# DrQuestion/monica

Hardware: AMD Instinct MI355X
Metric: reads/sec classified (higher is better)
Workload: dtype u32/u64 integer; int16 pairs in the alignment kernels (int32 / int8 in the long-call and literal ones); float32 islands: overlap ratio, MAPQ

## Files before the change

### include/monica_amd.h

```cpp
#ifndef MONICA_AMD_H
#define MONICA_AMD_H

#include <stdint.h>
#include <stddef.h>

#ifdef __cplusplus
extern "C" {
#endif

#define MNC_OK               0
#define MNC_ERR_ARG         (-1)
#define MNC_ERR_IO          (-2)
#define MNC_ERR_FORMAT      (-3)
#define MNC_ERR_NOMEM       (-4)
#define MNC_ERR_HIP         (-5)
#define MNC_ERR_NODEVICE    (-6)
#define MNC_ERR_UNSUPPORTED (-7)
#define MNC_ERR_RANGE       (-8)

#define MNC_UNMAPPED   (-1)
#define MNC_AMBIGUOUS  (-2)
#define MNC_SKIPPED    (-3)

typedef struct mnc_index  mnc_index;
// ... 96 lines not shown
#define MNC_STAGE_DP_POST     14
#define MNC_STAGE_DP_FILL     15
#define MNC_STAGE_DP_FILL_T1  16
#define MNC_STAGE_DP_FILL_T2  17
#define MNC_STAGE_DP_FILL_T3  18
#define MNC_STAGE_DP_EXT      19
#define MNC_STAGE_DP_FILL_TM  20
#define MNC_STAGE_DP_LFILL    21
#define MNC_N_STAGES          22
int mnc_engine_set_profiling(mnc_engine *eng, int on);
int mnc_engine_set_debug(mnc_engine *eng, int mode);
int mnc_engine_get_timings(mnc_engine *eng, double *ms, int64_t *launches, int reset);
const char *mnc_stage_name(int stage);
const char *mnc_stage_kernel(int stage);
int mnc_engine_get_counters(mnc_engine *eng, int64_t *c, int n);

int mnc_index_set_host_tables(mnc_index *idx, int on);
int mnc_index_set_region_bits(mnc_index *idx, int bits);
int mnc_engine_dump_tables(mnc_engine *eng, void *dst, int64_t cap_bytes, int64_t *n_bytes);

#define MNC_DUMP_MINIMIZERS 1
#define MNC_DUMP_MZ_OFFSETS 2
#define MNC_DUMP_ANCHORS    3
#define MNC_DUMP_AN_OFFSETS 4
#define MNC_DUMP_CHAIN_F    5
#define MNC_DUMP_CHAIN_P    6
#define MNC_DUMP_CHAIN_V    7
#define MNC_DUMP_REGS       8
#define MNC_DUMP_REG_OFFSETS 9
#define MNC_DUMP_REP_LEN    10
// ... 74 lines not shown
```

### monica_amd/_capi.py

```python
import ctypes as C
import os

import numpy as np

_HERE = os.path.dirname(os.path.abspath(__file__))
os.environ.setdefault("OMP_WAIT_POLICY", "passive")
LIB_PATH = os.environ.get("MONICA_AMD_LIB") or os.path.join(_HERE, "libmonica_amd.so")

OK = 0
ERR_ARG, ERR_IO, ERR_FORMAT, ERR_NOMEM, ERR_HIP, ERR_NODEVICE, ERR_UNSUPPORTED, ERR_RANGE = range(-1, -9, -1)
UNMAPPED = -1
AMBIGUOUS = -2
SKIPPED = -3

HIT_DTYPE = np.dtype([("rid", "<i4"), ("mapq", "<i4"), ("nm", "<i4"), ("mlen", "<i4")])
REG_DTYPE = np.dtype([("id", "<i4"), ("parent", "<i4"), ("rid", "<i4"), ("rev", "<i4"),
                      ("rs", "<i4"), ("re", "<i4"), ("qs", "<i4"), ("qe", "<i4"),
                      ("score", "<i4"), ("score0", "<i4"), ("cnt", "<i4"), ("as", "<i4"),
                      ("mlen", "<i4"), ("blen", "<i4"), ("subsc", "<i4"), ("n_sub", "<i4"),
                      ("mapq", "<i4"), ("hash", "<u4"),
                      ("dp_score", "<i4"), ("dp_max", "<i4"), ("dp_max2", "<i4"), ("n_ambi", "<i4"),
                      ("n_cigar", "<i4"), ("flags", "<i4")])
MZ_DTYPE = np.dtype([("hash", "<u4"), ("pos_strand", "<u4")])
ANCHOR_DTYPE = np.dtype([("x", "<u8"), ("y", "<u8")])
# ... 10 lines not shown
CONTRACT_DP, CONTRACT_CHAIN = 0, 1
MAX_READ_LEN = (1 << 20) - 1
MAX_READ_LEN_WIDE = (1 << 24) - 1
MAX_READS_WIDE = 1 << 16

EXPORTS = [
    "mnc_strerror", "mnc_last_error", "mnc_device_count", "mnc_device_name", "mnc_device_mem_info",
    "mnc_index_build", "mnc_index_build_mem", "mnc_index_build_device", "mnc_index_build_mem_device", "mnc_index_save", "mnc_index_save_mmi", "mnc_index_load", "mnc_index_free",
    "mnc_index_info", "mnc_index_contig_name", "mnc_index_contig_len", "mnc_index_contig_genome",
    "mnc_index_genome_name", "mnc_index_genome_len", "mnc_index_dump", "mnc_index_set_mid_occ",
    "mnc_engine_create", "mnc_engine_destroy", "mnc_engine_stream", "mnc_engine_device_bytes", "mnc_index_device_bytes", "mnc_engine_set_index",
    "mnc_classify_batch", "mnc_engine_prefetch", "mnc_engine_prefetch_cancel", "mnc_classify_device", "mnc_engine_sync", "mnc_engine_fetch_hits",
    "mnc_counts", "mnc_best_hit",
    "mnc_engine_set_profiling", "mnc_engine_set_debug", "mnc_engine_set_contract", "mnc_engine_set_long_reads", "mnc_index_set_host_tables", "mnc_index_set_region_bits", "mnc_engine_dump_tables",
    "mnc_comm_unique_id", "mnc_comm_init_rank", "mnc_comm_destroy", "mnc_comm_count", "mnc_allreduce_counts", "mnc_allgather_summaries", "mnc_shard_summary", "mnc_merge_summaries", "mnc_engine_get_timings", "mnc_stage_name", "mnc_stage_kernel",
    "mnc_engine_get_counters", "mnc_engine_dump",
    "mnc_fastq_open", "mnc_fastq_close", "mnc_fastq_next", "mnc_fastq_detach_batch", "mnc_fastq_remaining", "mnc_fastq_bases", "mnc_fastq_offsets",
    "mnc_fastq_quals", "mnc_fastq_title", "mnc_fastq_route",
    "mnc_hitmap_create", "mnc_hitmap_load", "mnc_hitmap_save", "mnc_hitmap_free", "mnc_hitmap_size",
    "mnc_hitmap_update", "mnc_hitmap_n_names", "mnc_hitmap_name", "mnc_host_alloc", "mnc_host_free", "mnc_host_set_io_workers",
    "mnc_synth_genome", "mnc_synth_diverge", "mnc_synth_reads", "mnc_synth_reads_device", "mnc_version",
]


class IndexInfo(C.Structure):
    _fields_ = [("k", C.c_int32), ("w", C.c_int32), ("n_contigs", C.c_int32), ("n_genomes", C.c_int32),
                ("mid_occ", C.c_int32), ("reserved", C.c_int32), ("n_keys", C.c_int64),
                ("n_occ", C.c_int64), ("total_len", C.c_int64), ("table_slots", C.c_int64),
                ("device_bytes", C.c_int64)]


# ... 52 lines not shown
    sig("mnc_engine_destroy", None, [vp])
    sig("mnc_engine_stream", vp, [vp])
    sig("mnc_engine_prefetch", i32, [vp, vp, vp, u32, C.POINTER(C.c_int)])
    sig("mnc_engine_prefetch_cancel", i32, [vp])
    sig("mnc_engine_set_index", i32, [vp, vp])
    sig("mnc_engine_device_bytes", i32, [vp, C.POINTER(C.c_int64)])
    sig("mnc_index_device_bytes", i32, [vp, i32, C.POINTER(C.c_int64)])
    sig("mnc_classify_batch", i32, [vp, vp, vp, u32, i32, vp, vp, vp])
    sig("mnc_classify_device", i32, [vp, vp, vp, u32, i64, i32, i32, vp, vp, vp, vp])
    sig("mnc_engine_sync", i32, [vp])
    sig("mnc_engine_fetch_hits", i32, [vp, vp, vp, i64, C.POINTER(i64)])
    sig("mnc_counts", i32, [vp, vp, vp, vp, u32, i32, vp])
    sig("mnc_best_hit", i32, [vp, i32, C.POINTER(i32)])
    sig("mnc_engine_set_profiling", i32, [vp, i32])
    sig("mnc_engine_set_debug", i32, [vp, i32])
    sig("mnc_index_set_host_tables", i32, [vp, i32])
    sig("mnc_index_set_region_bits", i32, [vp, i32])
    sig("mnc_engine_dump_tables", i32, [vp, vp, C.c_int64, vp])
    sig("mnc_engine_set_contract", i32, [vp, i32])
    sig("mnc_engine_set_long_reads", i32, [vp, i32])
    sig("mnc_comm_unique_id", i32, [vp])
    sig("mnc_comm_init_rank", i32, [vp, i32, i32, C.POINTER(vp)])
    sig("mnc_comm_destroy", i32, [vp])
    sig("mnc_comm_count", i32, [vp, C.POINTER(i32)])
    sig("mnc_allreduce_counts", i32, [vp, i32, vp, vp])
    sig("mnc_allgather_summaries", i32, [vp, vp, C.c_size_t, vp, vp])
    sig("mnc_shard_summary", i32, [vp, vp, vp, i64, i32, vp, vp])
    sig("mnc_merge_summaries", i32, [vp, i32, i64, vp, vp, vp, vp, vp])
    sig("mnc_engine_get_timings", i32, [vp, vp, vp, i32])
    sig("mnc_stage_name", cp, [i32])
# ... 318 lines not shown
        ln = np.zeros(N_STAGES, dtype=np.int64)
        check(lib().mnc_engine_get_timings(self._h, ms.ctypes.data, ln.ctypes.data, 1 if reset else 0))
        names = [lib().mnc_stage_name(s).decode() for s in range(N_STAGES)]
        return {names[s]: (float(ms[s]), int(ln[s])) for s in range(N_STAGES)}

    def counters(self):
        c = np.zeros(24, dtype=np.int64)
        check(lib().mnc_engine_get_counters(self._h, c.ctypes.data, 24))
        keys = ["minimizers", "probe_hits", "anchors", "chains", "regions", "gated_hits", "ambiguous_reads", "batch_redone",
                "dp_segments", "dp_fill_tier1", "dp_fill_tier2", "dp_fill_handed_back",
                "dp_fill_steps_t1", "dp_fill_steps_t2", "dp_fill_steps_t3", "dp_ext_cell_steps",
                "dp_literal_big", "dp_literal_mid", "dp_long_gaps", "dp_literal_big_handed_back", "dp_long_extensions", "dp_fill_tier3",
                "dp_fill_tier_mid", "dp_fill_steps_tm"]
        return dict(zip(keys, (int(x) for x in c)))

    def dump(self, what, dtype):
        n = C.c_int64(0)
        rc = lib().mnc_engine_dump(self._h, what, None, 0, C.byref(n))
        if rc not in (OK, ERR_RANGE):
            check(rc)
        buf = np.zeros(max(n.value, 1), dtype=np.uint8)
        check(lib().mnc_engine_dump(self._h, what, buf.ctypes.data, len(buf), C.byref(n)))
        return buf[:n.value].view(dtype).copy()


def best_hit(hits):
    arr = np.zeros(len(hits), dtype=HIT_DTYPE)
    for i, (nm, mlen) in enumerate(hits):
        arr[i]["nm"], arr[i]["mlen"] = nm, mlen
    out = C.c_int(0)
# ... 139 lines not shown
```

### monica_amd/csrc/engine.hip

```cpp
#include <hip/hip_runtime.h>
#include <algorithm>
#include <cmath>
#include <cstdio>
#include <cstring>
#include <cstdlib>
#include <new>
#include <vector>

#include "device.h"
#include <atomic>
#include <thread>

#include "scan.h"

namespace mnc {

void launch_pack(const Batch &B, hipStream_t st);
void launch_sketch(const Batch &B, hipStream_t st);
void launch_partition(const Batch &B, hipStream_t st);
int partition_prepare();
void launch_probe(const Batch &B, hipStream_t st);
void launch_collect(const Batch &B, hipStream_t st);
void launch_expand_sort(const Batch &B, const uint32_t *lists, const ClassSpans &spans, int NM, hipStream_t st);
int expand_sort_prepare(int max_nm);
void launch_backtrack(const Batch &B, const uint32_t *read_list, uint32_t n_list, hipStream_t st);
void launch_bin_reads(const Batch &B, const ChainClasses &C, uint32_t *cls_count, uint32_t *cls_list, hipStream_t st);
void launch_chain_dp_ring(const Batch &B, const uint32_t *lists, const ClassSpans &spans, int stress, hipStream_t st);
void launch_chain_tail(const Batch &B, const uint32_t *lists, const ClassSpans &spans, int NM, hipStream_t st);
size_t chain_tail_lds_bytes(int NM);
int chain_tail_prepare(size_t max_lds);

static const ChainClasses CHAIN_CLASSES = { 22, { 64, 128, 192, 256, 320, 384, 448, 512, 576, 640, 768, 896, 1024, 1280, 1536, 1792, 2048, 2560,
                                                  3072, 4096, 6144, 8192 } };
void launch_regions(const Batch &B, void *regx, uint64_t *k64a, uint64_t *k64b, mnc_hit_t *gated, hipStream_t st);
void launch_regions_post(const Batch &B, mnc_reg_t *work, void *regx, uint64_t *k64a, int32_t *tmp, mnc_hit_t *gated, hipStream_t st);
void launch_dp_gather(const Batch &B, hipStream_t st);
int dp_gather_long_prepare(int lds_anchors);
void launch_dp_gather_long(const Batch &B, const uint32_t *lists, const ClassSpans &spans, int lds_anchors, hipStream_t st);
void launch_dp_round(const Batch &B, int first, hipStream_t st);
void launch_dp_round_end(const Batch &B, hipStream_t st);
int dp_plan_prepare();
void launch_dp_plan(const Batch &B, const int32_t *work_list, unsigned max_work, int wave_form, int state_max, long long p_max, int cig_max,
                    long long big_state, long long big_p, long long big_cig, long long huge_state, long long huge_p, long long huge_cig, hipStream_t st);
size_t dp_align_ws_bytes(long long state_max, long long p_max, long long cig_max);
int dp_align_prepare(int lds_bytes);
int dp_stitch_prepare();
size_t dp_inv_ws_words(int max_gap);
void launch_dp_inv(const Batch &B, const int32_t *work_list, int32_t *next_list, int32_t *ws, int n_wg, hipStream_t st);
size_t dp_stitch_pool_slack(int n_wg);
void launch_dp_align(const Batch &B, uint8_t *ws, int n_wg, long long state_max, long long p_max, long long cig_max,
// ... 50 lines not shown
                                                             const int64_t *chunk_off_bm, int64_t *q_off)
{
	const uint32_t c = blockIdx.x, b = threadIdx.x, PB_N = blockDim.x;
	const uint32_t t0 = c * HC_TILES, t1 = min(n_tiles, t0 + HC_TILES);
	int64_t run = chunk_off_bm[(size_t)b * n_chunks + c];
	for (uint32_t t = t0; t < t1; ++t) {
		q_off[(size_t)t * PB_N + b] = run;
		run += hist_tm[(size_t)t * PB_N + b];
	}
	if (c == 0 && b == 0) q_off[(size_t)n_tiles * PB_N] = chunk_off_bm[(size_t)PB_N * n_chunks];
}

struct MailItem { const void *src; uint32_t dst_word, n_words; };
constexpr int MAIL_MAX = 8;
struct MailList { MailItem it[MAIL_MAX]; int n; };
__global__ __launch_bounds__(64) void mnc_mail(MailList L, uint32_t *host_box)
{
	for (int k = 0; k < L.n; ++k) {
		const uint32_t *s = static_cast<const uint32_t*>(L.it[k].src);
		for (uint32_t i = threadIdx.x; i < L.it[k].n_words; i += 64) host_box[L.it[k].dst_word + i] = s[i];
	}
	__threadfence_system();
}

struct Buf {
	void *p = nullptr;
	size_t cap = 0;
	int ensure(size_t bytes)
	{
		if (bytes <= cap) return MNC_OK;
		if (p) { (void)hipFree(p); p = nullptr; cap = 0; }
		size_t want = bytes + bytes / 8 + 256;
		hipError_t e = hipMalloc(&p, want);
		if (e != hipSuccess) { p = nullptr; set_error("hipMalloc(%zu) failed: %s", want, hipGetErrorString(e)); return MNC_ERR_NOMEM; }
		cap = want;
		return MNC_OK;
	}
// ... 244 lines not shown
	const int64_t *pf_offsets = nullptr;
	uint32_t pf_n = 0;
	int64_t pf_total = 0;
	Buf packed, mz, hits, hist_tm, q_off, qrec, bhits, bhit_cnt;
	size_t q_cap_override = 0;
	Buf ambig, skip, mz_cnt, hit_cnt, rep_len, an_cnt, an_off, n_chain, n_reg, scan_sums, hit_off, best_mlen, hist_sums, hist_offs;
	Buf a, f, p, v, t, u;
	Buf chains_tmp, regs, regx, k64a, k64b, tmp_i32, gated, hits_csr;
	Buf stats, cls_count, cls_list;
	int contract = MNC_CONTRACT_DP;
	Buf ca, ca_cnt, chain_dst, regdp, segs, cig_seg, cig_reg, dp_ctr, work_a, work_b, big_list, huge_list, reg_cnt, regs2;
	SharedWs *ws = nullptr;
	Buf fill1, fill2, fill3, fill_mid, fill_fb, plan_long, extp, mid_list, lfill, lext, bigfb, ext1, ext2, ext3, ext4, gen_list;
	size_t seg_cap_override = 0, cig_cap_override = 0;
	uint32_t *mailbox = nullptr;
	int last_redos = 0;
	long long prev_wide_calls = 0;
	int slot_pad = 2;
	Buf inv_ws;
	int cur_max_read_len = 0;
	int long_reads = 0;
	bool cur_wide = false;
	bool have_merged = false;
	std::vector<int64_t> merged_off;
	std::vector<mnc_hit_t> merged_hits;
	int64_t merged_ctr[24]{};
	int debug = 0;
	Batch B{};
	bool have_batch = false;
	int64_t last_total_anchors = 0, last_total_hits = -1;
// ... 156 lines not shown
	if (rc) { mnc_engine_destroy(e); return rc; }
	hipError_t he = hipSetDevice(device);
	int least = 0, greatest = 0;
	if (he == hipSuccess) {
		if (hipDeviceGetStreamPriorityRange(&least, &greatest) != hipSuccess) least = greatest = 0;
		he = hipStreamCreateWithPriority(&e->stream, hipStreamNonBlocking, greatest);
	}
	for (int k = 0; k < mnc_engine::N_SIDE && he == hipSuccess; ++k) {
		he = k < 3 ? hipStreamCreateWithFlags(&e->side[k], hipStreamNonBlocking) : hipStreamCreateWithPriority(&e->side[k], hipStreamNonBlocking, greatest);
		if (he == hipSuccess) he = hipEventCreateWithFlags(&e->ev_join[k], hipEventDisableTiming);
	}
	if (he == hipSuccess) he = hipEventCreateWithFlags(&e->ev_fork, hipEventDisableTiming);
	if (he == hipSuccess) he = hipEventCreateWithFlags(&e->ev_lfill, hipEventDisableTiming);
	if (he == hipSuccess) he = hipStreamCreateWithPriority(&e->copy_stream, hipStreamNonBlocking, least);
	if (he == hipSuccess) he = hipEventCreateWithFlags(&e->ev_prefetch, hipEventDisableTiming);
	if (he == hipSuccess) he = hipHostMalloc((void**)&e->mailbox, 1024, hipHostMallocDefault);
	if (he != hipSuccess) { set_error("stream creation failed: %s", hipGetErrorString(he)); mnc_engine_destroy(e); return MNC_ERR_HIP; }
	for (int s = 0; s < MNC_N_STAGES; ++s) for (int k = 0; k < 2; ++k) (void)hipEventCreate(&e->ev[s][k]);
	std::vector<int32_t> gap(GAP_LUT);
	const float avg_span = (float)idx->k;
	for (int dd = 0; dd < GAP_LUT; ++dd) {
		int lg = 0;
		for (uint32_t v = (uint32_t)dd; v >>= 1;) ++lg;
		gap[dd] = (int)(dd * .01 * avg_span) + (dd ? lg >> 1 : 0);
	}
	rc = e->gap_lut.ensure(GAP_LUT * 4);
	if (!rc) rc = logf_tables(e, 1 << 21);
	if (!rc) rc = e->dp_ctr.ensure(64 * 8);
	if (!rc) rc = dp_align_prepare(DP_LDS_BYTES);
	if (!rc) rc = e->stats.ensure(16 * 8);
	if (!rc) rc = e->cls_count.ensure((MAX_CHAIN_CLASSES + 1) * 4 + 64);
// ... 110 lines not shown
	e->contract = contract;
	return MNC_OK;
}

extern "C" int mnc_engine_set_long_reads(mnc_engine *e, int on)
{
	if (!e) return MNC_ERR_ARG;
	e->long_reads = on != 0;
	return MNC_OK;
}

extern "C" int mnc_engine_set_debug(mnc_engine *e, int on)
{
	if (!e) return MNC_ERR_ARG;
	e->debug = on;
	return MNC_OK;
}

extern "C" int mnc_engine_get_timings(mnc_engine *e, double *ms, int64_t *launches, int reset)
{
	if (!e) return MNC_ERR_ARG;
	for (int s = 0; s < MNC_N_STAGES; ++s) {
		if (ms) ms[s] = e->ms[s];
		if (launches) launches[s] = e->launches[s];
		if (reset) e->ms[s] = 0, e->launches[s] = 0;
	}
	return MNC_OK;
}

namespace {
// ... 55 lines not shown
	launch_dp_ext(B, 32, B.ext_list1, 16, 18, B.fill_fb, 12, e->ws->ext_p.as<uint8_t>(), DP_WG_EXT, s1);
	launch_dp_ext(B, 64, B.ext_list2, 17, 19, B.fill_fb, 12, e->ws->ext_p.as<uint8_t>(), DP_WG_EXT, s1);
	launch_dp_ext(B, 128, B.ext_list3, 24, 26, B.fill_fb, 12, e->ws->ext_p.as<uint8_t>(), DP_WG_EXT / 2, s1);
	launch_dp_ext(B, 256, B.ext_list4, 25, 27, B.fill_fb, 12, e->ws->ext_p.as<uint8_t>(), DP_WG_EXT / 4, s1);
	mark(MNC_STAGE_DP_EXT, 1);
	if (serial) {
		launch_dp_lext(B, B.lext_list, 62, 63, B.fill_fb, 12, e->ws->lext_p.as<uint8_t>(), DP_WG_LEXT, s0);
		long_passes(s0);
	}
	launch_dp_align(B, e->ws->dp_ws.as<uint8_t>(), 2 * DP_WG_SMALL, DP_STATE_SMALL, DP_P_SMALL, DP_CIG_SMALL, DP_LDS0_STATE, DP_LDS0_P, DP_LDS0_CIG, 0, s2);
}
static void align_rest(const Batch &B, mnc_engine *e, hipStream_t st)
{
	launch_dp_align(B, e->ws->dp_ws.as<uint8_t>(), DP_WG_SMALL, DP_STATE_SMALL, DP_P_SMALL, DP_CIG_SMALL, DP_LDS_BYTES, 0, 0, 2, st);
	launch_dp_align(B, e->ws->dp_ws_big.as<uint8_t>(), (dp_align_long_packed(B) && !(e->debug & 0x10000)) ? 64 : DP_WG_BIG, DP_STATE_BIG, DP_P_BIG, DP_CIG_BIG, DP_LDS_BYTES, 0, 0, 4, st);
}

static int classify_once(mnc_engine *e, const uint8_t *d_bases, const int64_t *d_offsets,
                         uint32_t n_reads, int64_t total_bases, int min_mapq,
                         int32_t *d_assign, mnc_hit_t *d_best, int32_t *d_nhits, int64_t *d_counts, int *overflowed)
{
	hipStream_t st = e->stream;
	const mnc_index *idx = e->idx;
	*overflowed = 0;
	const size_t nr = (size_t)n_reads, nb = (size_t)total_bases;
	const int pb_bits = e->didx->pb_bits;
	const size_t PB_N = (size_t)1 << pb_bits, PS_TILES = (size_t)(e->cur_wide ? PS_TILES_MIN / 2 : PS_TILES_MIN);
	const size_t n_tiles = (nr + PT_READS - 1) / PT_READS, n_super = (n_tiles + PS_TILES - 1) / PS_TILES;
	size_t q_cap = nb / 3 + 4096;
	if (e->q_cap_override > q_cap) q_cap = e->q_cap_override < nb + 4096 ? e->q_cap_override : nb + 4096;
// ... 41 lines not shown
		while ((1LL << rb) < (int64_t)idx->contig_name.size()) ++rb;
		while ((1LL << pb) < longest) ++pb;
		const bool fits = 1 + rb + pb + 21 <= 64;
		B.rid_bits = fits ? rb : 0, B.rpos_bits = fits ? pb : 0;
	}
	const MapParams &P = idx->par;
	B.min_cnt = P.min_cnt, B.min_sc = P.min_chain_score, B.bw = P.bw, B.max_gap = P.max_gap, B.max_skip = P.max_chain_skip;
	B.max_iter = P.max_chain_iter, B.best_n = P.best_n, B.seed = P.seed, B.max_join_long = P.max_join_long;
	B.max_join_short = P.max_join_short, B.min_join_flank_sc = P.min_join_flank_sc, B.mask_level = P.mask_level;
	B.pri_ratio = P.pri_ratio, B.min_join_flank_ratio = P.min_join_flank_ratio;
	B.gap_lut = e->gap_lut.as<int32_t>(), B.logf_lut = e->logf_lut.as<float>(), B.logf_a_lut = e->logf_a_lut.as<float>(), B.logf_n = e->logf_n;
	B.debug_route = (e->debug >> 17 & 15) | ((e->debug >> 22 & 1) << 4) | ((e->debug >> 5 & 1) << 5)
	              | ((e->debug >> 6 & 1) << 6) | ((e->debug >> 7 & 1) << 7)
	              | ((e->debug >> 3 & 1) << 8) | ((e->debug & 1) << 9)
	              | (((unsigned)e->debug >> 31 & 1) << 10);
	B.fill_pred = (e->debug >> 8 & 0xff) ? (e->debug >> 8 & 0xff) : 32;
	B.fill_pred_mid = (e->debug >> 24 & 0x7f) ? (e->debug >> 24 & 0x7f) : 34;
	B.fill_pred_auto = !(e->debug >> 8 & 0xff) && !(e->debug >> 24 & 0x7f) && P.a == 2 && P.b == 4 && P.q == 4 && P.e == 2 &&
	                   P.q2 == 24 && P.e2 == 1 && !getenv("MNC_FILL_PRED_FIXED");
	B.contract = e->contract, B.seq4 = e->didx->seq4, B.seq_off = e->didx->seq_off;
	B.sc_a = P.a, B.sc_b = P.b, B.gap_q = P.q, B.gap_e = P.e, B.gap_q2 = P.q2, B.gap_e2 = P.e2, B.sc_ambi = P.sc_ambi;
	B.zdrop = P.zdrop, B.zdrop_inv = P.zdrop_inv, B.end_bonus = P.end_bonus, B.min_dp_max = P.min_dp_max, B.min_ksw_len = P.min_ksw_len;
	B.max_sw_mat = P.max_sw_mat;
	B.packed = e->packed.as<uint32_t>(), B.ambig = e->ambig.as<uint32_t>(), B.skip = e->skip.as<uint32_t>(), B.mz = e->mz.as<uint2>(), B.hits = e->hits.as<HitRec>();
	B.mz_cnt = e->mz_cnt.as<int32_t>(), B.hit_cnt = e->hit_cnt.as<int32_t>(), B.rep_len = e->rep_len.as<int32_t>();
	B.an_cnt = e->an_cnt.as<int64_t>(), B.an_off = e->an_off.as<int64_t>(), B.n_chain = e->n_chain.as<int32_t>(), B.n_reg = e->n_reg.as<int32_t>(), B.best_mlen = e->best_mlen.as<int32_t>();
	B.n_tiles = (uint32_t)n_tiles, B.n_super = (uint32_t)n_super;
	B.hist_tm = e->hist_tm.as<uint32_t>(), B.q_off = e->q_off.as<int64_t>(), B.qrec = e->qrec.as<uint64_t>();
	B.q_cap = (int64_t)q_cap, B.bhits = e->bhits.as<HitRec>(), B.bhit_cnt = e->bhit_cnt.as<uint32_t>();
	B.overflow = reinterpret_cast<uint32_t*>(e->stats.as<int64_t>() + 8);
	B.assign = d_assign, B.best = d_best, B.nhits = d_nhits ? d_nhits : e->out_nhits.as<int32_t>(), B.counts = d_counts;
	B.stats = e->stats.as<int64_t>();

	HIP_TRY(hipMemsetAsync(B.ambig, 0, (nr + 1) * 4, st));
	HIP_TRY(hipMemsetAsync(B.skip, 0, (nr + 1) * 4, st));
	HIP_TRY(hipMemsetAsync(B.packed + nb / 16, 0, 16, st));
	HIP_TRY(hipMemsetAsync(B.overflow, 0, 8, st));

	{ StageTimer t(e, MNC_STAGE_PACK);   launch_pack(B, st); }
	{ StageTimer t(e, MNC_STAGE_SKETCH); launch_sketch(B, st); }
	{
		StageTimer t(e, MNC_STAGE_PARTITION);
		{
			const uint32_t n_chunks = (uint32_t)((n_tiles + HC_TILES - 1) / HC_TILES);
			uint32_t *sums_bm = e->hist_sums.as<uint32_t>();
			int64_t *off_bm = e->hist_offs.as<int64_t>();
			hipLaunchKernelGGL(mnc_hist_chunk_sums, dim3(n_chunks), dim3((unsigned)PB_N), 0, st, B.hist_tm, (uint32_t)n_tiles, n_chunks, sums_bm);
			exclusive_scan(ScanInPlain<uint32_t>{sums_bm}, (int64_t)n_chunks * PB_N, off_bm, e->scan_sums.as<int64_t>(), st);
			hipLaunchKernelGGL(mnc_hist_offsets, dim3(n_chunks), dim3((unsigned)PB_N), 0, st, B.hist_tm, (uint32_t)n_tiles, n_chunks, off_bm, B.q_off);
		}
		launch_partition(B, st);
	}
	{ StageTimer t(e, MNC_STAGE_PROBE);   launch_probe(B, st); }
	{ StageTimer t(e, MNC_STAGE_COLLECT); launch_collect(B, st); }
	HIP_TRY(hipGetLastError());
	int64_t total_anchors = 0, total_q = 0;
	uint32_t cls_count[MAX_CHAIN_CLASSES + 1] = {0}, overflow = 0;
	{
		StageTimer t(e, MNC_STAGE_SORT);
		exclusive_scan(ScanInPlain<int64_t>{B.an_cnt}, (int64_t)n_reads, B.an_off, e->scan_sums.as<int64_t>(), st);
		HIP_TRY(hipMemsetAsync(e->cls_count.p, 0, (MAX_CHAIN_CLASSES + 1) * 4, st));
		launch_bin_reads(B, CHAIN_CLASSES, e->cls_count.as<uint32_t>(), e->cls_list.as<uint32_t>(), st);
		MailList ml;
		ml.n = 4;
		ml.it[0] = { B.an_off + n_reads, 0, 2 }, ml.it[1] = { B.q_off + n_tiles * PB_N, 2, 2 };
		ml.it[2] = { e->cls_count.p, 4, (uint32_t)(MAX_CHAIN_CLASSES + 1) }, ml.it[3] = { B.overflow, 4 + MAX_CHAIN_CLASSES + 1, 1 };
		hipLaunchKernelGGL(mnc_mail, dim3(1), dim3(64), 0, st, ml, e->mailbox);
		HIP_TRY(hipStreamSynchronize(st));
		memcpy(&total_anchors, e->mailbox, 8), memcpy(&total_q, e->mailbox + 2, 8);
		memcpy(cls_count, e->mailbox + 4, (MAX_CHAIN_CLASSES + 1) * 4);
		overflow = e->mailbox[4 + MAX_CHAIN_CLASSES + 1];
	}
	if (overflow || total_q > (int64_t)q_cap) {
		e->q_cap_override = (size_t)total_q + (size_t)total_q / 8 + 4096;
		*overflowed = 1;
		return MNC_OK;
	}
	if (total_anchors < 0 || total_anchors >= (1LL << 31) * 16) { set_error("anchor count %lld out of range", (long long)total_anchors); return MNC_ERR_UNSUPPORTED; }
	e->last_total_anchors = total_anchors;
	const size_t na = (size_t)total_anchors + 4, ns = (size_t)total_anchors / 3 + 4, nsr = ns + nr * (size_t)e->slot_pad;
	ENS(a, na * sizeof(Anchor));
	ENS(f, na * 4); ENS(p, na * 4); ENS(v, na * 4); ENS(t, na * 4);
	ENS(u, na * 8);
// ... 91 lines not shown
		ENSW(dp_ws, ws_small * DP_WG_SMALL * 2); ENSW(dp_ws_big, ws_big * DP_WG_BIG); ENSW(dp_ws_bigfb, ws_big * DP_WG_BIGFB); ENSW(dp_ws_huge, ws_huge * DP_WG_HUGE); ENS2(huge_list, seg_cap * 4); ENSW(dp_ws_mid, ws_small * DP_WG_MID); ENS2(mid_list, seg_cap * 4); ENS2(lfill, seg_cap * 4); ENSW(lfill_p, dp_lfill_p_slot() * DP_WG_LFILL); ENS2(lext, seg_cap * 4); ENS2(bigfb, seg_cap * 4); ENSW(lext_p, dp_lext_p_slot() * DP_WG_LEXT);
		ENS2(plan_long, (nr * 4 + 1024) * 4);
		ENS2(fill1, seg_cap * 4); ENS2(fill2, seg_cap * 4); ENS2(fill3, seg_cap * 4); ENS2(fill_mid, seg_cap * 4); ENS2(fill_fb, seg_cap * 4); ENSW(fill_p, dp_fillp_slot() * DP_WG_FILL); ENSW(fill_cig, dp_fillp_cig_slot() * DP_WG_FILL); ENS2(extp, seg_cap * 4 * 8); ENSW(extp_p, dp_extp_slot() * DP_WG_EXT); ENSW(extp_cig, dp_extp_cig_slot() * DP_WG_EXT); ENS2(ext1, seg_cap * 4); ENS2(ext2, seg_cap * 4); ENS2(ext3, seg_cap * 4); ENS2(ext4, seg_cap * 4); ENS2(gen_list, seg_cap * 4); ENSW(ext_p, dp_fill_p_slot() * DP_WG_EXT);
#undef ENS2
		if (rc2) return rc2;
		B.ca = e->ca.as<Anchor>(), B.ca_cnt = e->ca_cnt.as<int32_t>(), B.chain_dst = e->chain_dst.as<int32_t>(), B.regdp = e->regdp.as<RegDP>();
		B.segs = e->segs.as<Seg>(), B.seg_cap = (int64_t)seg_cap, B.cig_seg = e->cig_seg.as<uint32_t>(), B.cig_reg = e->cig_reg.as<uint32_t>();
		B.cig_seg_cap = (int64_t)cig_cap, B.cig_reg_cap = (int64_t)cig_reg_cap, B.dp_ctr = e->dp_ctr.as<unsigned long long>();
		B.big_list = e->big_list.as<int32_t>(), B.huge_list = e->huge_list.as<int32_t>(), B.reg_cnt = e->reg_cnt.as<int32_t>();
		B.plan_long_list = e->plan_long.as<int32_t>(), B.plan_long_cap = (long long)(nr * 4 + 1024);
		B.fill_list1 = e->fill1.as<int32_t>(), B.fill_list2 = e->fill2.as<int32_t>(), B.fill_list3 = e->fill3.as<int32_t>(), B.fill_list_mid = e->fill_mid.as<int32_t>(), B.fill_fb = e->fill_fb.as<int32_t>();
		B.ext_list1 = e->ext1.as<int32_t>(), B.ext_list2 = e->ext2.as<int32_t>(), B.ext_list3 = e->ext3.as<int32_t>(), B.ext_list4 = e->ext4.as<int32_t>(), B.gen_list = e->gen_list.as<int32_t>(), B.extp_list = e->extp.as<int32_t>(), B.mid_list = e->mid_list.as<int32_t>(), B.lfill_list = e->lfill.as<int32_t>(), B.lext_list = e->lext.as<int32_t>(), B.bigfb_list = e->bigfb.as<int32_t>();
		B.lds0_state = DP_LDS0_STATE, B.lds0_p = DP_LDS0_P, B.lds0_cig = DP_LDS0_CIG;
		int32_t *lists[2] = { e->work_a.as<int32_t>(), e->work_b.as<int32_t>() };
		B.next_list = lists[0];
		HIP_TRY(hipMemsetAsync(e->dp_ctr.p, 0, 64 * 8, st));
		{ StageTimer t(e, MNC_STAGE_REGIONS);   launch_regions(B, e->regx.p, e->k64a.as<uint64_t>(), e->k64b.as<uint64_t>(), e->gated.as<mnc_hit_t>(), st); }
		{
			StageTimer t(e, MNC_STAGE_DP_PLAN);
			launch_dp_gather(B, st);
			int c0 = 0;
			while (c0 < CHAIN_CLASSES.n && CHAIN_CLASSES.nm[c0] <= 1024) ++c0;
			ClassSpans sp;
			sp.n = CHAIN_CLASSES.n + 1 - c0, sp.stride = (uint32_t)n_reads, sp.start[0] = 0;
			for (int c = c0; c <= CHAIN_CLASSES.n; ++c) sp.start[c - c0 + 1] = sp.start[c - c0] + cls_count[c];
			launch_dp_gather_long(B, e->cls_list.as<uint32_t>() + (size_t)c0 * n_reads, sp, CHAIN_CLASSES.nm[CHAIN_CLASSES.n - 1], st);
		}
		unsigned max_work = (unsigned)nsr;
		const int long_reads = (e->debug & 0x10) ? 2 : (e->debug & 0x800000) ? 0 : n_reads <= 4096 ? 2
		                     : (e->cur_max_read_len <= 0 || e->cur_max_read_len > 6144) ? 1 : 0;
		for (int round = 0;; ++round) {
			const int32_t *work = lists[round & 1];
			int32_t *next = lists[(round + 1) & 1];
			B.next_list = next;
			launch_dp_round(B, round == 0, st);
			if (round == 0) {
				{ StageTimer t(e, MNC_STAGE_DP_PLAN);   launch_dp_plan(B, work, max_work, long_reads, (int)DP_STATE_SMALL, DP_P_SMALL, (int)DP_CIG_SMALL, DP_STATE_BIG, DP_P_BIG, DP_CIG_BIG, DP_STATE_HUGE, DP_P_HUGE, DP_CIG_HUGE, st); }
				{
					StageTimer t(e, MNC_STAGE_DP_FILL);
					if (int rcf = fork()) return rcf;
					if (e->debug & 0x10000) align_round(B, e, e->side[0], e->side[0], e->side[0], e->side[0], e->side[0]);
					else align_round(B, e, e->side[0], e->side[1], st, e->side[2], e->side[3]);
					if (int rcj = join()) return rcj;
				}
				{
					StageTimer t(e, MNC_STAGE_DP_ALIGN);
					align_rest(B, e, st);
				}
				{ StageTimer t(e, MNC_STAGE_DP_STITCH); launch_dp_stitch(B, work, next, (e->debug & 0x200000) ? 0 : e->cur_max_read_len > 0 ? e->cur_max_read_len : 8192, DP_WG_STITCH, st); }
			} else {
// ... 1 lines not shown
				if (int rcf = fork()) return rcf;
				if (e->debug & 0x10000) align_round(B, e, e->side[0], e->side[0], e->side[0], e->side[0], e->side[0]);
				else align_round(B, e, e->side[0], e->side[1], st, e->side[2], e->side[3]);
				if (int rcj = join()) return rcj;
				align_rest(B, e, st);
				launch_dp_stitch(B, work, next, (e->debug & 0x200000) ? 0 : e->cur_max_read_len > 0 ? e->cur_max_read_len : 8192, DP_WG_STITCH, st);
				launch_dp_inv(B, work, next, e->inv_ws.as<int32_t>(), (int)std::min<unsigned>(DP_WG_INV, max_work), st);
			}
			launch_dp_round_end(B, st);
			unsigned long long ctr[6] = {0};
			{
				MailList ml;
				ml.n = 3;
				ml.it[0] = { e->dp_ctr.p, 0, 12 };
				ml.it[1] = { e->dp_ctr.as<unsigned long long>() + 6, 12, 2 }, ml.it[2] = { e->dp_ctr.as<unsigned long long>() + 58, 14, 2 };
				hipLaunchKernelGGL(mnc_mail, dim3(1), dim3(64), 0, st, ml, e->mailbox);
				HIP_TRY(hipStreamSynchronize(st));
				memcpy(ctr, e->mailbox, sizeof(ctr));
				if (round == 0 && n_reads >= 4096) {
					unsigned long long big = 0, huge = 0;
					memcpy(&big, e->mailbox + 12, 8), memcpy(&huge, e->mailbox + 14, 8);
					e->prev_wide_calls = (long long)(big + huge);
				}
			}
			if (ctr[4] != 0) {
				if (ctr[4] >= 9) { set_error("a gap between two seeds is too large for the alignment workspace"); return MNC_ERR_UNSUPPORTED; }
				if (ctr[4] == 5) {
					e->slot_pad = e->slot_pad * 4;
					*overflowed = 2;
					return MNC_OK;
				}
				e->seg_cap_override = na + 2 * ns + 1024;
				e->cig_cap_override = cig_cap * 4;
				*overflowed = 2;
				return MNC_OK;
			}
			if (ctr[5] == 0) break;
			if (round > 256) { set_error("base-level alignment does not settle"); return MNC_ERR_HIP; }
			max_work = (unsigned)ctr[5];
		}
		{ StageTimer t(e, MNC_STAGE_DP_POST); launch_regions_post(B, e->regs2.as<mnc_reg_t>(), e->regx.p, e->k64a.as<uint64_t>(), e->tmp_i32.as<int32_t>(), e->gated.as<mnc_hit_t>(), st); }
	} else {
		StageTimer t(e, MNC_STAGE_REGIONS);
		launch_regions(B, e->regx.p, e->k64a.as<uint64_t>(), e->k64b.as<uint64_t>(), e->gated.as<mnc_hit_t>(), st);
	}
	HIP_TRY(hipGetLastError());
	e->have_batch = true;
	return MNC_OK;
}

extern "C" int mnc_classify_device(mnc_engine *e, const uint8_t *d_bases, const int64_t *d_offsets,
                                   uint32_t n_reads, int64_t total_bases, int max_read_len, int min_mapq,
                                   int32_t *d_assign, mnc_hit_t *d_best, int32_t *d_nhits, int64_t *d_counts)
{
	if (!e || !d_offsets || !d_assign || (total_bases > 0 && !d_bases) || total_bases < 0) return MNC_ERR_ARG;
	if (((uintptr_t)d_bases & 15u) != 0) { set_error("d_bases must be 16-byte aligned"); return MNC_ERR_ARG; }
// ... 6 lines not shown
	if (wide && n_reads > (uint32_t)WIDE_MAX_READS) { set_error("at most 2^16 reads in a call with reads of 2^20 bases or more (wide query records hold a 16-bit read ordinal)"); return MNC_ERR_UNSUPPORTED; }
	if (total_bases >= (1LL << 40)) return MNC_ERR_UNSUPPORTED;
	HIP_TRY(hipSetDevice(e->device));
	e->have_batch = false, e->last_total_hits = -1, e->have_merged = false, e->cur_wide = wide;
	const int64_t logf_want = wide ? std::min<int64_t>((int64_t)e->idx->par.a * max_read_len + 1024, INT32_MAX / 8) : 1 << 21;
	if (logf_want > e->logf_n) {
		HIP_TRY(hipStreamSynchronize(e->stream));
		if (int lrc = logf_tables(e, (int)logf_want)) return lrc;
	}
	if (n_reads == 0) {
		memset(&e->B, 0, sizeof(e->B));
		e->have_batch = true, e->last_total_anchors = 0;
		return MNC_OK;
	}
	int overflowed = 0, q_redone = 0, dp_redone = 0;
	e->cur_max_read_len = max_read_len, e->last_redos = 0;
	int rc = MNC_OK;
	for (;;) {
		rc = classify_once(e, d_bases, d_offsets, n_reads, total_bases, min_mapq, d_assign, d_best, d_nhits, d_counts, &overflowed);
		if (rc || !overflowed) break;
		++e->last_redos;
		if (overflowed == 1 && ++q_redone > 1) { set_error("query record budget exceeded twice"); rc = MNC_ERR_NOMEM; break; }
		if (overflowed == 2 && ++dp_redone > 6) { set_error("segment / CIGAR pools of the alignment stage exceeded after %d enlargements", dp_redone - 1); rc = MNC_ERR_NOMEM; break; }
	}
	return rc;
}

extern "C" int mnc_engine_prefetch(mnc_engine *e, const uint8_t *bases, const int64_t *offsets, uint32_t n_reads, int *started)
{
	if (!e || !offsets || !started) return MNC_ERR_ARG;
	*started = 0;
// ... 363 lines not shown
```

### monica_amd/csrc/k_post.hip

```cpp
#include "device.h"

namespace mnc {

__device__ __forceinline__ uint64_t mix64(uint64_t key)
{
	key = ~key + (key << 21);
	key = key ^ key >> 24;
	key = (key + (key << 3)) + (key << 8);
	key = key ^ key >> 14;
	key = (key + (key << 2)) + (key << 4);
	key = key ^ key >> 28;
	key = key + (key << 31);
	return key;
}

__device__ __forceinline__ uint32_t wang32(uint32_t key)
{
	key += ~(key << 15);
	key ^=  (key >> 10);
	key +=  (key << 3);
	key ^=  (key >> 6);
	key += ~(key << 11);
	key ^=  (key >> 16);
	return key;
// ... 400 lines not shown
					d.read = (int32_t)rd, d.order = i << 8, d.state = 1;
					B.regdp[slot + i] = d;
					B.next_list[w0 + i] = (int32_t)(slot + i);
				}
			}
		}
	} else if (dp) B.ca_cnt[rd] = 0;
	if (dp) { B.reg_cnt[rd] = n_regs; return; }
	B.n_reg[rd] = n_regs;
	B.assign[rd] = assign;
	if (B.best) B.best[rd] = best;
	B.nhits[rd] = nhits;
	B.best_mlen[rd] = best.mlen;
}

__global__ __launch_bounds__(64) void mnc_regions_post(Batch B, mnc_reg_t *work_all, RegX *regx_all, uint64_t *k64a_all,
                                                       int32_t *tmp_all, mnc_hit_t *gated_all)
{
	const uint32_t rd = blockIdx.x * blockDim.x + threadIdx.x;
	if (rd >= B.n_reads) return;
	int32_t assign = MNC_UNMAPPED, nhits = 0;
	mnc_hit_t best;
	best.rid = best.mapq = best.nm = best.mlen = 0;
	const int n0 = B.reg_cnt[rd];
	int n_regs = 0;
	if (n0 > 0) {
		const int64_t slot = reg_slot(B, rd);
		mnc_reg_t *src = B.regs + slot, *r = work_all + slot;
		RegX *ex = regx_all + slot;
		uint64_t *ka = k64a_all + slot;
		int32_t *w = tmp_all + slot * 4, *tmp = w + n0;
		mnc_hit_t *gated = gated_all + slot;
		for (int i = 0; i < n0; ++i) w[i] = i;
// ... 41 lines not shown
		for (int i = 0; i < n_regs; ++i) src[i] = r[i], B.regdp[slot + i].cig_off = (int64_t)ex[i].x0, B.regdp[slot + i].n_cigar = r[i].n_cigar;
	}
	if (B.skip[rd]) {
		assign = MNC_SKIPPED, nhits = 0;
		memset(&best, 0, sizeof(best));
	}
	B.n_reg[rd] = n_regs;
	B.assign[rd] = assign;
	if (B.best) B.best[rd] = best;
	B.nhits[rd] = nhits;
	B.best_mlen[rd] = best.mlen;
}

constexpr int CT_THREADS = 256, CT_READS = 4096, CT_LDS_BINS = 3 * 1024;

__global__ __launch_bounds__(CT_THREADS) void mnc_count_taxa(Batch B)
{
	__shared__ unsigned long long s_bins[CT_LDS_BINS];
	const int n_bins = B.n_genomes * 3;
	const bool in_lds = n_bins <= CT_LDS_BINS;
	if (in_lds) {
		for (int k = threadIdx.x; k < n_bins; k += CT_THREADS) s_bins[k] = 0;
		__syncthreads();
	}
	unsigned long long *bins = in_lds ? s_bins : (unsigned long long*)B.counts;
	const uint32_t lo = blockIdx.x * CT_READS;
	const uint32_t hi = min(B.n_reads, lo + CT_READS);
	for (uint32_t rd = lo + threadIdx.x; rd < hi; rd += CT_THREADS) {
		const int a = B.assign[rd];
		if (a < 0) continue;
		const int g = B.contig_genome[a];
		atomicAdd(&bins[g * 3 + 0], 1ULL);
// ... 13 lines not shown
	const uint32_t rd = blockIdx.x * blockDim.x + threadIdx.x;
	if (rd >= B.n_reads) return;
	const int n = B.nhits[rd];
	if (n == 0) return;
	const mnc_hit_t *src = gated_all + reg_slot(B, rd);
	mnc_hit_t *dst = out + hit_off[rd];
	for (int i = 0; i < n; ++i) dst[i] = src[i];
}

void launch_regions(const Batch &B, void *regx, uint64_t *k64a, uint64_t *k64b, mnc_hit_t *gated, hipStream_t st)
{
	if (B.n_reads == 0) return;
	hipLaunchKernelGGL(mnc_regions_decide, dim3((B.n_reads + 63) / 64), dim3(64), 0, st, B,
	                   reinterpret_cast<RegX*>(regx), k64a, k64b, gated);
	if (B.counts && B.contract != MNC_CONTRACT_DP)
		hipLaunchKernelGGL(mnc_count_taxa, dim3((B.n_reads + CT_READS - 1) / CT_READS), dim3(CT_THREADS), 0, st, B);
}

void launch_regions_post(const Batch &B, mnc_reg_t *work, void *regx, uint64_t *k64a, int32_t *tmp, mnc_hit_t *gated, hipStream_t st)
{
	if (B.n_reads == 0) return;
	hipLaunchKernelGGL(mnc_regions_post, dim3((B.n_reads + 63) / 64), dim3(64), 0, st, B, work,
	                   reinterpret_cast<RegX*>(regx), k64a, tmp, gated);
	if (B.counts) hipLaunchKernelGGL(mnc_count_taxa, dim3((B.n_reads + CT_READS - 1) / CT_READS), dim3(CT_THREADS), 0, st, B);
}

void launch_gather_hits(const Batch &B, const mnc_hit_t *gated, const int64_t *hit_off, mnc_hit_t *out, hipStream_t st)
{
	if (B.n_reads == 0) return;
	hipLaunchKernelGGL(mnc_gather_hits, dim3((B.n_reads + 255) / 256), dim3(256), 0, st, B, gated, hit_off, out);
}

}
```

Baseline: 2.886 million.

## Replace host stream syncs with mailbox sequence polling and speculative post launch

The mail kernel now writes a sequence number with a system-scope release store, and the host spin-polls that word instead of calling hipStreamSynchronize, falling back to a stream sync after a timeout. Four separate memset calls are folded into a single clear kernel. The regions-post and count-taxa kernels are launched speculatively before each DP round's host wait and exit early unless the round has settled, so the final post work is already queued when the loop ends. This cuts host-device round-trip latency and launch overhead, at the cost of a busy-waiting CPU thread and extra no-op kernel launches on rounds that have not settled.

```diff
diff --git a/include/monica_amd.h b/include/monica_amd.h
--- a/include/monica_amd.h
+++ b/include/monica_amd.h
@@ -134,6 +134,7 @@
 const char *mnc_stage_name(int stage);
 const char *mnc_stage_kernel(int stage);
 int mnc_engine_get_counters(mnc_engine *eng, int64_t *c, int n);
+int mnc_engine_host_waits(mnc_engine *eng, int64_t *w, int n);
 
 int mnc_index_set_host_tables(mnc_index *idx, int on);
 int mnc_index_set_region_bits(mnc_index *idx, int bits);
diff --git a/monica_amd/_capi.py b/monica_amd/_capi.py
--- a/monica_amd/_capi.py
+++ b/monica_amd/_capi.py
@@ -48,7 +48,7 @@
     "mnc_counts", "mnc_best_hit",
     "mnc_engine_set_profiling", "mnc_engine_set_debug", "mnc_engine_set_contract", "mnc_engine_set_long_reads", "mnc_index_set_host_tables", "mnc_index_set_region_bits", "mnc_engine_dump_tables",
     "mnc_comm_unique_id", "mnc_comm_init_rank", "mnc_comm_destroy", "mnc_comm_count", "mnc_allreduce_counts", "mnc_allgather_summaries", "mnc_shard_summary", "mnc_merge_summaries", "mnc_engine_get_timings", "mnc_stage_name", "mnc_stage_kernel",
-    "mnc_engine_get_counters", "mnc_engine_dump",
+    "mnc_engine_get_counters", "mnc_engine_host_waits", "mnc_engine_dump",
     "mnc_fastq_open", "mnc_fastq_close", "mnc_fastq_next", "mnc_fastq_detach_batch", "mnc_fastq_remaining", "mnc_fastq_bases", "mnc_fastq_offsets",
     "mnc_fastq_quals", "mnc_fastq_title", "mnc_fastq_route",
     "mnc_hitmap_create", "mnc_hitmap_load", "mnc_hitmap_save", "mnc_hitmap_free", "mnc_hitmap_size",
@@ -131,6 +131,8 @@
     sig("mnc_best_hit", i32, [vp, i32, C.POINTER(i32)])
     sig("mnc_engine_set_profiling", i32, [vp, i32])
     sig("mnc_engine_set_debug", i32, [vp, i32])
+    if hasattr(L, "mnc_engine_host_waits"):
+        sig("mnc_engine_host_waits", i32, [vp, vp, i32])
     sig("mnc_index_set_host_tables", i32, [vp, i32])
     sig("mnc_index_set_region_bits", i32, [vp, i32])
     sig("mnc_engine_dump_tables", i32, [vp, vp, C.c_int64, vp])
@@ -479,6 +481,11 @@
                 "dp_fill_tier_mid", "dp_fill_steps_tm"]
         return dict(zip(keys, (int(x) for x in c)))
 
+    def host_waits(self):
+        w = np.zeros(3, dtype=np.int64)
+        check(lib().mnc_engine_host_waits(self._h, w.ctypes.data, 3))
+        return {"polled": int(w[0]), "synced": int(w[1]), "rounds": int(w[2])}
+
     def dump(self, what, dtype):
         n = C.c_int64(0)
         rc = lib().mnc_engine_dump(self._h, what, None, 0, C.byref(n))
diff --git a/monica_amd/csrc/engine.hip b/monica_amd/csrc/engine.hip
--- a/monica_amd/csrc/engine.hip
+++ b/monica_amd/csrc/engine.hip
@@ -9,6 +9,7 @@
 
 #include "device.h"
 #include <atomic>
+#include <chrono>
 #include <thread>
 
 #include "scan.h"
@@ -33,7 +34,7 @@
 static const ChainClasses CHAIN_CLASSES = { 22, { 64, 128, 192, 256, 320, 384, 448, 512, 576, 640, 768, 896, 1024, 1280, 1536, 1792, 2048, 2560,
                                                   3072, 4096, 6144, 8192 } };
 void launch_regions(const Batch &B, void *regx, uint64_t *k64a, uint64_t *k64b, mnc_hit_t *gated, hipStream_t st);
-void launch_regions_post(const Batch &B, mnc_reg_t *work, void *regx, uint64_t *k64a, int32_t *tmp, mnc_hit_t *gated, hipStream_t st);
+void launch_regions_post(const Batch &B, mnc_reg_t *work, void *regx, uint64_t *k64a, int32_t *tmp, mnc_hit_t *gated, int if_settled, hipStream_t st);
 void launch_dp_gather(const Batch &B, hipStream_t st);
 int dp_gather_long_prepare(int lds_anchors);
 void launch_dp_gather_long(const Batch &B, const uint32_t *lists, const ClassSpans &spans, int lds_anchors, hipStream_t st);
@@ -114,13 +115,26 @@
 struct MailItem { const void *src; uint32_t dst_word, n_words; };
 constexpr int MAIL_MAX = 8;
 struct MailList { MailItem it[MAIL_MAX]; int n; };
-__global__ __launch_bounds__(64) void mnc_mail(MailList L, uint32_t *host_box)
+constexpr uint32_t MAIL_WORDS = 256, MAIL_SEQ = MAIL_WORDS - 1;
+__global__ __launch_bounds__(64) void mnc_mail(MailList L, uint32_t *host_box, uint32_t seq)
 {
 	for (int k = 0; k < L.n; ++k) {
 		const uint32_t *s = static_cast<const uint32_t*>(L.it[k].src);
 		for (uint32_t i = threadIdx.x; i < L.it[k].n_words; i += 64) host_box[L.it[k].dst_word + i] = s[i];
 	}
 	__threadfence_system();
+	__syncthreads();
+	if (threadIdx.x == 0) __hip_atomic_store(host_box + MAIL_SEQ, seq, __ATOMIC_RELEASE, __HIP_MEMORY_SCOPE_SYSTEM);
+}
+
+struct ClearItem { uint32_t *p; uint32_t n_words; };
+constexpr int CLEAR_MAX = 8;
+struct ClearList { ClearItem it[CLEAR_MAX]; int n; };
+__global__ __launch_bounds__(256) void mnc_clear(ClearList L)
+{
+	const uint32_t t = blockIdx.x * 256 + threadIdx.x, step = gridDim.x * 256;
+	for (int k = 0; k < L.n; ++k)
+		for (uint32_t i = t; i < L.it[k].n_words; i += step) L.it[k].p[i] = 0;
 }
 
 struct Buf {
@@ -395,6 +409,9 @@
 	Buf fill1, fill2, fill3, fill_mid, fill_fb, plan_long, extp, mid_list, lfill, lext, bigfb, ext1, ext2, ext3, ext4, gen_list;
 	size_t seg_cap_override = 0, cig_cap_override = 0;
 	uint32_t *mailbox = nullptr;
+	uint32_t mail_seq = 0;
+	int last_rounds = 0;
+	int64_t mail_polled = 0, mail_synced = 0;
 	int last_redos = 0;
 	long long prev_wide_calls = 0;
 	int slot_pad = 2;
@@ -581,7 +598,8 @@
 	if (he == hipSuccess) he = hipEventCreateWithFlags(&e->ev_lfill, hipEventDisableTiming);
 	if (he == hipSuccess) he = hipStreamCreateWithPriority(&e->copy_stream, hipStreamNonBlocking, least);
 	if (he == hipSuccess) he = hipEventCreateWithFlags(&e->ev_prefetch, hipEventDisableTiming);
-	if (he == hipSuccess) he = hipHostMalloc((void**)&e->mailbox, 1024, hipHostMallocDefault);
+	if (he == hipSuccess) he = hipHostMalloc((void**)&e->mailbox, MAIL_WORDS * 4, hipHostMallocDefault);
+	if (he == hipSuccess) memset(e->mailbox, 0, MAIL_WORDS * 4);
 	if (he != hipSuccess) { set_error("stream creation failed: %s", hipGetErrorString(he)); mnc_engine_destroy(e); return MNC_ERR_HIP; }
 	for (int s = 0; s < MNC_N_STAGES; ++s) for (int k = 0; k < 2; ++k) (void)hipEventCreate(&e->ev[s][k]);
 	std::vector<int32_t> gap(GAP_LUT);
@@ -722,6 +740,14 @@
 {
 	if (!e) return MNC_ERR_ARG;
 	e->debug = on;
+	return MNC_OK;
+}
+
+extern "C" int mnc_engine_host_waits(mnc_engine *e, int64_t *w, int n)
+{
+	if (!e || !w || n < 2) return MNC_ERR_ARG;
+	w[0] = e->mail_polled, w[1] = e->mail_synced;
+	if (n >= 3) w[2] = e->last_rounds;
 	return MNC_OK;
 }
 
@@ -807,6 +833,32 @@
 {
 	launch_dp_align(B, e->ws->dp_ws.as<uint8_t>(), DP_WG_SMALL, DP_STATE_SMALL, DP_P_SMALL, DP_CIG_SMALL, DP_LDS_BYTES, 0, 0, 2, st);
 	launch_dp_align(B, e->ws->dp_ws_big.as<uint8_t>(), (dp_align_long_packed(B) && !(e->debug & 0x10000)) ? 64 : DP_WG_BIG, DP_STATE_BIG, DP_P_BIG, DP_CIG_BIG, DP_LDS_BYTES, 0, 0, 4, st);
+}
+
+constexpr int DEBUG_HOST_SYNC = 0x8000;
+constexpr long long MAIL_SPIN_NS = 250LL * 1000 * 1000;
+
+static uint32_t mail_send(mnc_engine *e, const MailList &ml, hipStream_t st)
+{
+	const uint32_t seq = ++e->mail_seq ? e->mail_seq : ++e->mail_seq;
+	hipLaunchKernelGGL(mnc_mail, dim3(1), dim3(64), 0, st, ml, e->mailbox, seq);
+	return seq;
+}
+static int mail_wait(mnc_engine *e, uint32_t seq, hipStream_t st)
+{
+	if (!(e->debug & DEBUG_HOST_SYNC)) {
+		const auto t0 = std::chrono::steady_clock::now();
+		for (unsigned spin = 1;; ++spin) {
+			if (__atomic_load_n(e->mailbox + MAIL_SEQ, __ATOMIC_ACQUIRE) == seq) { ++e->mail_polled; return MNC_OK; }
+			if ((spin & 1023) == 0 && std::chrono::duration_cast<std::chrono::nanoseconds>(std::chrono::steady_clock::now() - t0).count() > MAIL_SPIN_NS) break;
+#if defined(__x86_64__) || defined(__i386__)
+			__builtin_ia32_pause();
+#endif
+		}
+	}
+	HIP_TRY(hipStreamSynchronize(st));
+	++e->mail_synced;
+	return MNC_OK;
 }
 
 static int classify_once(mnc_engine *e, const uint8_t *d_bases, const int64_t *d_offsets,
@@ -878,9 +930,9 @@
 	              | ((e->debug >> 6 & 1) << 6) | ((e->debug >> 7 & 1) << 7)
 	              | ((e->debug >> 3 & 1) << 8) | ((e->debug & 1) << 9)
 	              | (((unsigned)e->debug >> 31 & 1) << 10);
-	B.fill_pred = (e->debug >> 8 & 0xff) ? (e->debug >> 8 & 0xff) : 32;
+	B.fill_pred = (e->debug >> 8 & 0x7f) ? (e->debug >> 8 & 0x7f) : 32;
 	B.fill_pred_mid = (e->debug >> 24 & 0x7f) ? (e->debug >> 24 & 0x7f) : 34;
-	B.fill_pred_auto = !(e->debug >> 8 & 0xff) && !(e->debug >> 24 & 0x7f) && P.a == 2 && P.b == 4 && P.q == 4 && P.e == 2 &&
+	B.fill_pred_auto = !(e->debug >> 8 & 0x7f) && !(e->debug >> 24 & 0x7f) && P.a == 2 && P.b == 4 && P.q == 4 && P.e == 2 &&
 	                   P.q2 == 24 && P.e2 == 1 && !getenv("MNC_FILL_PRED_FIXED");
 	B.contract = e->contract, B.seq4 = e->didx->seq4, B.seq_off = e->didx->seq_off;
 	B.sc_a = P.a, B.sc_b = P.b, B.gap_q = P.q, B.gap_e = P.e, B.gap_q2 = P.q2, B.gap_e2 = P.e2, B.sc_ambi = P.sc_ambi;
@@ -896,10 +948,20 @@
 	B.assign = d_assign, B.best = d_best, B.nhits = d_nhits ? d_nhits : e->out_nhits.as<int32_t>(), B.counts = d_counts;
 	B.stats = e->stats.as<int64_t>();
 
-	HIP_TRY(hipMemsetAsync(B.ambig, 0, (nr + 1) * 4, st));
-	HIP_TRY(hipMemsetAsync(B.skip, 0, (nr + 1) * 4, st));
-	HIP_TRY(hipMemsetAsync(B.packed + nb / 16, 0, 16, st));
-	HIP_TRY(hipMemsetAsync(B.overflow, 0, 8, st));
+	const bool host_sync = (e->debug & DEBUG_HOST_SYNC) != 0;
+	if (host_sync) {
+		HIP_TRY(hipMemsetAsync(B.ambig, 0, (nr + 1) * 4, st));
+		HIP_TRY(hipMemsetAsync(B.skip, 0, (nr + 1) * 4, st));
+		HIP_TRY(hipMemsetAsync(B.packed + nb / 16, 0, 16, st));
+		HIP_TRY(hipMemsetAsync(B.overflow, 0, 8, st));
+	} else {
+		ClearList cl;
+		cl.n = 5;
+		cl.it[0] = { B.ambig, (uint32_t)nr + 1 }, cl.it[1] = { B.skip, (uint32_t)nr + 1 }, cl.it[2] = { B.packed + nb / 16, 4 };
+		cl.it[3] = { B.overflow, 2 }, cl.it[4] = { e->cls_count.as<uint32_t>(), (uint32_t)(MAX_CHAIN_CLASSES + 1) };
+		if (e->contract == MNC_CONTRACT_DP) cl.it[cl.n++] = { e->dp_ctr.as<uint32_t>(), 64 * 2 };
+		hipLaunchKernelGGL(mnc_clear, dim3((unsigned)std::min<size_t>(256, (nr + 256) / 256)), dim3(256), 0, st, cl);
+	}
 
 	{ StageTimer t(e, MNC_STAGE_PACK);   launch_pack(B, st); }
 	{ StageTimer t(e, MNC_STAGE_SKETCH); launch_sketch(B, st); }
@@ -923,14 +985,13 @@
 	{
 		StageTimer t(e, MNC_STAGE_SORT);
 		exclusive_scan(ScanInPlain<int64_t>{B.an_cnt}, (int64_t)n_reads, B.an_off, e->scan_sums.as<int64_t>(), st);
-		HIP_TRY(hipMemsetAsync(e->cls_count.p, 0, (MAX_CHAIN_CLASSES + 1) * 4, st));
+		if (host_sync) HIP_TRY(hipMemsetAsync(e->cls_count.p, 0, (MAX_CHAIN_CLASSES + 1) * 4, st));
 		launch_bin_reads(B, CHAIN_CLASSES, e->cls_count.as<uint32_t>(), e->cls_list.as<uint32_t>(), st);
 		MailList ml;
 		ml.n = 4;
 		ml.it[0] = { B.an_off + n_reads, 0, 2 }, ml.it[1] = { B.q_off + n_tiles * PB_N, 2, 2 };
 		ml.it[2] = { e->cls_count.p, 4, (uint32_t)(MAX_CHAIN_CLASSES + 1) }, ml.it[3] = { B.overflow, 4 + MAX_CHAIN_CLASSES + 1, 1 };
-		hipLaunchKernelGGL(mnc_mail, dim3(1), dim3(64), 0, st, ml, e->mailbox);
-		HIP_TRY(hipStreamSynchronize(st));
+		if (int rcm = mail_wait(e, mail_send(e, ml, st), st)) return rcm;
 		memcpy(&total_anchors, e->mailbox, 8), memcpy(&total_q, e->mailbox + 2, 8);
 		memcpy(cls_count, e->mailbox + 4, (MAX_CHAIN_CLASSES + 1) * 4);
 		overflow = e->mailbox[4 + MAX_CHAIN_CLASSES + 1];
@@ -1052,7 +1113,7 @@
 		B.lds0_state = DP_LDS0_STATE, B.lds0_p = DP_LDS0_P, B.lds0_cig = DP_LDS0_CIG;
 		int32_t *lists[2] = { e->work_a.as<int32_t>(), e->work_b.as<int32_t>() };
 		B.next_list = lists[0];
-		HIP_TRY(hipMemsetAsync(e->dp_ctr.p, 0, 64 * 8, st));
+		if (host_sync) HIP_TRY(hipMemsetAsync(e->dp_ctr.p, 0, 64 * 8, st));
 		{ StageTimer t(e, MNC_STAGE_REGIONS);   launch_regions(B, e->regx.p, e->k64a.as<uint64_t>(), e->k64b.as<uint64_t>(), e->gated.as<mnc_hit_t>(), st); }
 		{
 			StageTimer t(e, MNC_STAGE_DP_PLAN);
@@ -1072,6 +1133,7 @@
 			int32_t *next = lists[(round + 1) & 1];
 			B.next_list = next;
 			launch_dp_round(B, round == 0, st);
+			e->last_rounds = round + 1;
 			if (round == 0) {
 				{ StageTimer t(e, MNC_STAGE_DP_PLAN);   launch_dp_plan(B, work, max_work, long_reads, (int)DP_STATE_SMALL, DP_P_SMALL, (int)DP_CIG_SMALL, DP_STATE_BIG, DP_P_BIG, DP_CIG_BIG, DP_STATE_HUGE, DP_P_HUGE, DP_CIG_HUGE, st); }
 				{
@@ -1103,8 +1165,12 @@
 				ml.n = 3;
 				ml.it[0] = { e->dp_ctr.p, 0, 12 };
 				ml.it[1] = { e->dp_ctr.as<unsigned long long>() + 6, 12, 2 }, ml.it[2] = { e->dp_ctr.as<unsigned long long>() + 58, 14, 2 };
-				hipLaunchKernelGGL(mnc_mail, dim3(1), dim3(64), 0, st, ml, e->mailbox);
-				HIP_TRY(hipStreamSynchronize(st));
+				const uint32_t seq = mail_send(e, ml, st);
+				if (!host_sync) {
+					StageTimer t(e, MNC_STAGE_DP_POST);
+					launch_regions_post(B, e->regs2.as<mnc_reg_t>(), e->regx.p, e->k64a.as<uint64_t>(), e->tmp_i32.as<int32_t>(), e->gated.as<mnc_hit_t>(), 1, st);
+				}
+				if (int rcm = mail_wait(e, seq, st)) return rcm;
 				memcpy(ctr, e->mailbox, sizeof(ctr));
 				if (round == 0 && n_reads >= 4096) {
 					unsigned long long big = 0, huge = 0;
@@ -1128,7 +1194,7 @@
 			if (round > 256) { set_error("base-level alignment does not settle"); return MNC_ERR_HIP; }
 			max_work = (unsigned)ctr[5];
 		}
-		{ StageTimer t(e, MNC_STAGE_DP_POST); launch_regions_post(B, e->regs2.as<mnc_reg_t>(), e->regx.p, e->k64a.as<uint64_t>(), e->tmp_i32.as<int32_t>(), e->gated.as<mnc_hit_t>(), st); }
+		if (host_sync) { StageTimer t(e, MNC_STAGE_DP_POST); launch_regions_post(B, e->regs2.as<mnc_reg_t>(), e->regx.p, e->k64a.as<uint64_t>(), e->tmp_i32.as<int32_t>(), e->gated.as<mnc_hit_t>(), 0, st); }
 	} else {
 		StageTimer t(e, MNC_STAGE_REGIONS);
 		launch_regions(B, e->regx.p, e->k64a.as<uint64_t>(), e->k64b.as<uint64_t>(), e->gated.as<mnc_hit_t>(), st);
@@ -1165,7 +1231,7 @@
 		return MNC_OK;
 	}
 	int overflowed = 0, q_redone = 0, dp_redone = 0;
-	e->cur_max_read_len = max_read_len, e->last_redos = 0;
+	e->cur_max_read_len = max_read_len, e->last_redos = 0, e->last_rounds = 0;
 	int rc = MNC_OK;
 	for (;;) {
 		rc = classify_once(e, d_bases, d_offsets, n_reads, total_bases, min_mapq, d_assign, d_best, d_nhits, d_counts, &overflowed);
diff --git a/monica_amd/csrc/k_post.hip b/monica_amd/csrc/k_post.hip
--- a/monica_amd/csrc/k_post.hip
+++ b/monica_amd/csrc/k_post.hip
@@ -438,9 +438,12 @@
 	B.best_mlen[rd] = best.mlen;
 }
 
+__device__ __forceinline__ bool round_settled(const Batch &B) { return (B.dp_ctr[4] | B.dp_ctr[5]) == 0; }
+
 __global__ __launch_bounds__(64) void mnc_regions_post(Batch B, mnc_reg_t *work_all, RegX *regx_all, uint64_t *k64a_all,
-                                                       int32_t *tmp_all, mnc_hit_t *gated_all)
-{
+                                                       int32_t *tmp_all, mnc_hit_t *gated_all, int if_settled)
+{
+	if (if_settled && !round_settled(B)) return;
 	const uint32_t rd = blockIdx.x * blockDim.x + threadIdx.x;
 	if (rd >= B.n_reads) return;
 	int32_t assign = MNC_UNMAPPED, nhits = 0;
@@ -512,8 +515,9 @@
 
 constexpr int CT_THREADS = 256, CT_READS = 4096, CT_LDS_BINS = 3 * 1024;
 
-__global__ __launch_bounds__(CT_THREADS) void mnc_count_taxa(Batch B)
-{
+__global__ __launch_bounds__(CT_THREADS) void mnc_count_taxa(Batch B, int if_settled)
+{
+	if (if_settled && !round_settled(B)) return;
 	__shared__ unsigned long long s_bins[CT_LDS_BINS];
 	const int n_bins = B.n_genomes * 3;
 	const bool in_lds = n_bins <= CT_LDS_BINS;
@@ -557,15 +561,15 @@
 	hipLaunchKernelGGL(mnc_regions_decide, dim3((B.n_reads + 63) / 64), dim3(64), 0, st, B,
 	                   reinterpret_cast<RegX*>(regx), k64a, k64b, gated);
 	if (B.counts && B.contract != MNC_CONTRACT_DP)
-		hipLaunchKernelGGL(mnc_count_taxa, dim3((B.n_reads + CT_READS - 1) / CT_READS), dim3(CT_THREADS), 0, st, B);
-}
-
-void launch_regions_post(const Batch &B, mnc_reg_t *work, void *regx, uint64_t *k64a, int32_t *tmp, mnc_hit_t *gated, hipStream_t st)
+		hipLaunchKernelGGL(mnc_count_taxa, dim3((B.n_reads + CT_READS - 1) / CT_READS), dim3(CT_THREADS), 0, st, B, 0);
+}
+
+void launch_regions_post(const Batch &B, mnc_reg_t *work, void *regx, uint64_t *k64a, int32_t *tmp, mnc_hit_t *gated, int if_settled, hipStream_t st)
 {
 	if (B.n_reads == 0) return;
 	hipLaunchKernelGGL(mnc_regions_post, dim3((B.n_reads + 63) / 64), dim3(64), 0, st, B, work,
-	                   reinterpret_cast<RegX*>(regx), k64a, tmp, gated);
-	if (B.counts) hipLaunchKernelGGL(mnc_count_taxa, dim3((B.n_reads + CT_READS - 1) / CT_READS), dim3(CT_THREADS), 0, st, B);
+	                   reinterpret_cast<RegX*>(regx), k64a, tmp, gated, if_settled);
+	if (B.counts) hipLaunchKernelGGL(mnc_count_taxa, dim3((B.n_reads + CT_READS - 1) / CT_READS), dim3(CT_THREADS), 0, st, B, if_settled);
 }
 
 void launch_gather_hits(const Batch &B, const mnc_hit_t *gated, const int64_t *hit_off, mnc_hit_t *out, hipStream_t st)
```

Result: no change. 2.891 million, median of 2 (+0.2%).
